# curioloop/rafting

Measured on AMD Instinct MI355X. Metric: raft-group decisions/sec (AppendEntries+vote), higher is better.
Workload: dtype int64

## Files before the change

### rafting_amd/csrc/rg_step.hpp

```cpp
#pragma once
#include "rg_device.hpp"
#include "rg_tier1n.hpp"

namespace rg {

typedef uint32_t u32x2 __attribute__((vector_size(8)));
typedef uint32_t u32x4 __attribute__((vector_size(16)));

template <class T> __device__ __forceinline__ T nt_load16(const T *p)
{
    static_assert(sizeof(T) == 16, "16-byte row");
    const u32x4 v = __builtin_nontemporal_load(reinterpret_cast<const u32x4 *>(p));
    T r; __builtin_memcpy(&r, &v, 16); return r;
}
template <class T> __device__ __forceinline__ T nt_load8(const T *p)
{
    static_assert(sizeof(T) == 8, "8-byte row");
    const u32x2 v = __builtin_nontemporal_load(reinterpret_cast<const u32x2 *>(p));
    T r; __builtin_memcpy(&r, &v, 8); return r;
}
template <class T> __device__ __forceinline__ void nt_store16(T *p, const T &x)
{
    static_assert(sizeof(T) == 16, "16-byte row");
    u32x4 v; __builtin_memcpy(&v, &x, 16);
// ... 535 lines not shown
                      c = (int64_t)sh_ev[slot][EV_C][lane], d = (int64_t)sh_ev[slot][EV_D][lane];
        int64_t e0 = (int64_t)(int32_t)aux;
        if constexpr (!EV32) e0 = (int64_t)sh_ev[slot][EV_E0][lane];
        const uint32_t kind = RG_HDR_KIND(hdr);
        { const int64_t top = *sh_flush; *sh_flush = ((kind == RG_EV_LOG_FLUSH) & (a > top)) ? a : top; }
        const bool skip = blocked & (kind != RG_EV_NONE);
        const bool done = tier1<F, int64_t, PeersWide<F>>(p, g, pe, st.fx, FAST & !skip, hdr, aux, a, b, c, d, e0);
        bool slow = !done & !skip;
        if (skip) st.fx = Fx{0u, RG_SKIPPED_AFTER_NEED_HOST, 0, 0};
        if (__builtin_amdgcn_ballot_w64(slow) != 0) {
            if (slow) slow = !tier15w<F, int64_t, PeersWide<F>>(p, g, pe, st.fx, FAST, hdr, aux, EV32 ? false : ((RG_HDR_HINT(hdr) != 0) & (p.hint != nullptr)), a, b, c, d, e0);
            if (slow) {
                int64_t hx = 0, hy = 0, e1 = e0, e2 = e0, e3 = e0;
                if constexpr (!EV32) {
                    hx = (int64_t)sh_ev[slot][EV_HX][lane]; hy = (int64_t)sh_ev[slot][EV_HY][lane];
                    e1 = (int64_t)sh_ev[slot][EV_E1][lane]; e2 = (int64_t)sh_ev[slot][EV_E2][lane]; e3 = (int64_t)sh_ev[slot][EV_E3][lane];
                }
                const Entries en = entries_of<EV32>(p, hdr, aux, e0, e1, e2, e3);
                const bool hinted = EV32 ? false : ((RG_HDR_HINT(hdr) != 0) & (p.hint != nullptr));
                st.run(hdr, aux, a, b, c, d, hinted, hx, hy, en, entries_readable(p, en, aux, RG_HDR_N(hdr)));
            }
        }
        const uint32_t status = st.fx.status, flags = st.fx.flags;
        if (status == RG_NEED_HOST) blocked = true;
        const uint32_t flags_all = flags | ((uint32_t)g.role << RG_F_ROLE_SHIFT) | (status << RG_F_STATUS_SHIFT);
        sh_out[slot][OUT_RESP][lane] = (flags & RG_F_REPLIED) ? (uint64_t)st.fx.resp_term : 0ull;
        sh_out[slot][OUT_FLAGS][lane] = (uint64_t)flags_all | ((uint64_t)g.role_epoch << 32);
        sh_out[slot][OUT_COMMIT][lane] = (uint64_t)g.commit;
        sh_out[slot][OUT_FROM][lane] = (uint64_t)st.fx.log_from;
        sh_out[slot][OUT_TERM][lane] = (uint64_t)g.term;
        sh_out[slot][OUT_VOTE][lane] = (uint64_t)(uint32_t)g.voted_for | ((uint64_t)(uint32_t)g.role << 32);
        lds_barrier();
    }
    uint32_t gi_out = gi;
    RG_FRESH_VGPR(gi_out);
    if (active) store_group(p.t, gi_out, g, pe, F);
    if (const int64_t at = sh_flush[1]; at != 0) {
        RG_GLOBAL_AS int64_t *slot = reinterpret_cast<RG_GLOBAL_AS int64_t *>((uint64_t)at);
        const int64_t top = sh_flush[0], window = sh_flush[2];
        if (top - window > *slot) *slot = top - window;
    }
}

template <int F, bool SPARSE>
__global__ __launch_bounds__(2 * BLOCK) void step_split_kernel(const StepParams p)
{
    __shared__ alignas(16) unsigned char smem[SplitLds<F, false>::BYTES];
    split_body<F, SPARSE, false>(p, smem);
}

struct Row32 { U32x2 h; I32x4 q; };

constexpr int CW_AUXC = 18;
template <int F = 0>
__device__ __forceinline__ uint32_t class_entry(const StepParams &p, uint32_t idx)
{
    const uint32_t kind = idx & 15u, slot = idx >> 4;
    const uint32_t P = (uint32_t)p.cluster, self = (uint32_t)p.self;
    const bool peer_ok = (slot < P) & (slot != self);
    const bool ack = (kind == RG_EV_AE_ACK) & peer_ok, vreq = (kind == RG_EV_RV_REQ) | (kind == RG_EV_PV_REQ),
               vrep = (kind == RG_EV_RV_REPLY) | (kind == RG_EV_PV_REPLY);
    const uint32_t j = ack ? (slot < self ? slot : slot - 1u) : 0u;
    const uint32_t cls = (ack ? 1u << CW_ACK : 0u) | (((kind == RG_EV_AE_REQ) & (slot < P)) ? 1u << CW_AE : 0u) | ((kind == RG_EV_CLIENT_APPEND) ? 1u << CW_CLIENT : 0u) |
                         (((ack | (kind == RG_EV_IS_ACK)) & peer_ok) ? 1u << CW_ACKANY : 0u) |
                         ((kind - (uint32_t)RG_EV_RV_REQ <= (uint32_t)(RG_EV_TIMEOUT - RG_EV_RV_REQ)) ? 1u << CW_ELK : 0u) |
                         ((vrep & peer_ok) ? 1u << CW_VR : 0u) | ((kind == RG_EV_PV_REPLY) ? 1u << CW_PV : 0u) | ((kind == RG_EV_TIMEOUT) ? 1u << CW_TO : 0u) |
                         ((vreq & (slot < P)) ? 1u << CW_VQ : 0u) | ((kind == RG_EV_PV_REQ) ? 1u << CW_PVQ : 0u) | ((kind == RG_EV_NONE) ? 1u << CW_NONE : 0u) |
                         ((((0x1CCu >> kind) & 1u) != 0) ? 1u << CW_AUXC : 0u);
    const uint32_t j4 = F > 6 ? (j & 15u) : j;
    return cls | (j4 << 10) | (slot << 5) | (31u - j);
}
__device__ __forceinline__ I32x4 class_word(const uint32_t *lutc, const Row32 &x)
{
    const uint32_t hdr = x.h.x, aux = x.h.y;
    const uint32_t e = lutc[hdr & 0xFFu];
    const int32_t n = (int32_t)(hdr >> 12);
    const sw same = (int32_t)(hdr << (31 - 10));
    const int32_t n_lim = (same >> 31) & (int32_t)RG_MAX_AE_ENTRIES;
    const sw ae_bad = ~s_pos(x.q.z) | s_lt(n_lim, n), cli_bad = s_lt(n, 1);
    const uint32_t auxm = (uint32_t)(((int32_t)(e << (31 - CW_AUXC)) | ((int32_t)(e << (31 - CW_AE)) & same)) >> 31);
    const uint32_t w = (uint32_t)x.q.x | (uint32_t)x.q.y | (uint32_t)x.q.z | (uint32_t)x.q.w | (aux & auxm);
    const uint32_t ood = (uint32_t)((int32_t)(w | (w << 1)) >> 31);
    const uint32_t off = (((uint32_t)ae_bad & 0x80000000u) >> (31 - CW_AE)) | (((uint32_t)cli_bad & 0x80000000u) >> (31 - CW_CLIENT)) | (1u << CW_AUXC) |
                         (ood & 0xFFF80000u);
    const uint32_t cw = (e & ~off) | ((hdr & 0x100u) << (CW_FLAG - 8));
    return I32x4{(int32_t)cw, (int32_t)aux, n, (int32_t)(hdr | (ood & KIND_OUT_OF_DOMAIN))};
}
__device__ __forceinline__ uint32_t expand_by_table(const uint32_t *lutm, const uint16_t *lute, uint32_t w)
{
    const uint32_t fast = lutm[w & 127u] | (uint32_t)lute[(w >> 7) & 127u];
    return ((int32_t)w < 0) ? (w & 0x00FFFFFFu) : fast;
}

template <int F, bool SPARSE, bool OUT32, int IOW = 1, int RPB = 1>
__device__ __forceinline__ bool narrow_body(const StepParams &p, unsigned char *smem)
{
    static_assert(RPB == 1 || (RPB == 2 && IOW == 1), "two rounds per hand-over: the two-wavefront workgroup only");
    constexpr int NO = 2 * RPB;
    typedef SplitLds<F, true, NO> L;
    I32x4 *sh_rec = reinterpret_cast<I32x4 *>(smem + L::N_REC);
    int32_t *sh_mv = reinterpret_cast<int32_t *>(smem + L::N_MV);
    I32x4 (*sh_evh)[BLOCK] = reinterpret_cast<I32x4 (*)[BLOCK]>(smem + L::N_EVH);
    I32x4 (*sh_evq)[BLOCK] = reinterpret_cast<I32x4 (*)[BLOCK]>(smem + L::N_EVQ);
    I32x4 (*sh_o0)[BLOCK] = reinterpret_cast<I32x4 (*)[BLOCK]>(smem + L::N_O0);
    I32x4 (*sh_o1)[BLOCK] = reinterpret_cast<I32x4 (*)[BLOCK]>(smem + L::N_O1);
    uint32_t *sh_bail = reinterpret_cast<uint32_t *>(smem + L::N_BAIL);
    uint32_t *sh_lutc = reinterpret_cast<uint32_t *>(smem + L::N_LUTC), *sh_lutm = reinterpret_cast<uint32_t *>(smem + L::N_LUTM);
    uint16_t *sh_lute = reinterpret_cast<uint16_t *>(smem + L::N_LUTE);
    uint32_t *sh_luts = reinterpret_cast<uint32_t *>(smem + L::N_LUTS);

    const uint32_t lane = threadIdx.x & (BLOCK - 1);
    const bool io_wave = __builtin_amdgcn_readfirstlane(threadIdx.x) >= (uint32_t)BLOCK;
    const uint32_t i = blockIdx.x * BLOCK + lane;
    const bool active = i < p.count;
    const uint32_t ir = active ? i : p.count - 1u;
    const uint32_t last_round = p.rounds - 1u;

    if (io_wave) {
        RG_HWID_BEGIN(1);
        const bool do_pub = IOW == 1 || __builtin_amdgcn_readfirstlane(threadIdx.x) < 2u * BLOCK;
        const bool do_ret = IOW == 1 || !do_pub;
        uint64_t b_head = reinterpret_cast<uint64_t>(p.head), b_q = reinterpret_cast<uint64_t>(p.abcd32),
                 b_reply = OUT32 ? reinterpret_cast<uint64_t>(p.out32) : reinterpret_cast<uint64_t>(p.reply),
                 b_logfx = reinterpret_cast<uint64_t>(p.logfx),
                 b_persist = OUT32 ? reinterpret_cast<uint64_t>(p.persist32) : reinterpret_cast<uint64_t>(p.persist);
        RG_OWN_SGPRS(b_head); RG_OWN_SGPRS(b_q); RG_OWN_SGPRS(b_reply); RG_OWN_SGPRS(b_logfx); RG_OWN_SGPRS(b_persist);
        const uint64_t round_rows = SPARSE ? p.stride : p.count;
        const uint32_t irm = ir & 0x0FFFFFFFu;
        int64_t io_base = 0;
        if constexpr (!OUT32) io_base = (p.has_bases != 0) ? p.t.ibase[SPARSE ? p.gid[ir] : ir] : 0;
        auto fetch = [&](uint32_t r, Row32 &x) {
            const uint64_t rb = (uint64_t)(r < p.rounds ? r : last_round) * round_rows;
            x.h = nt_load_at<U32x2>(b_head + rb * 8u, irm);
            x.q = nt_load_at<I32x4>(b_q + rb * 16u, irm);
        };
#pragma unroll
        for (int k = 0; k < 4; k++) sh_lutc[lane + 64u * k] = class_entry<F>(p, lane + 64u * k);
#pragma unroll
        for (int k = 0; k < 2; k++) {
            const uint32_t i7 = lane + 64u * k;
            sh_lutm[i7] = expand_predicates(i7);
            sh_lute[i7] = (uint16_t)(expand_predicates((i7 << 7) | 0x42u) & 0xFFFFu);
        }
        sh_luts[lane] = Tally::status_entry(lane);
        __builtin_amdgcn_wave_barrier();
        auto publish = [&](uint32_t slot, const Row32 &x) {
            sh_evh[slot][lane] = class_word(sh_lutc, x);
            sh_evq[slot][lane] = x.q;
        };
        Tally tally;
        auto retire = [&](uint32_t r, uint32_t hdr) {
            const uint32_t slot = r & (uint32_t)(NO - 1);
            const uint64_t rb16 = (uint64_t)r * round_rows * 16u;
            const I32x4 o0 = sh_o0[slot][lane], o1 = sh_o1[slot][lane];
            const uint32_t flags_all = expand_by_table(sh_lutm, sh_lute, (uint32_t)o0.y) | ((uint32_t)o1.w << RG_F_ROLE_SHIFT), flags = flags_all & 0xFFFFu, status = RG_F_STATUS(flags_all);
            if constexpr (OUT32) {
                nt_store_at(b_reply + rb16, irm, I32x4{(flags & RG_F_REPLIED) ? o0.x : 0, (int32_t)flags_all, o0.w, o1.x});
                if ((flags & RG_F_PERSIST) != 0) nt_store_at(b_persist + rb16, irm, I32x4{o1.y, o1.z, o0.z, o1.w});
            } else {
                rg_reply_t rep;
                rep.resp_term = (flags & RG_F_REPLIED) ? (int64_t)(uint32_t)o0.x : 0; rep.flags = flags_all; rep.role_epoch = (uint32_t)o0.z;
                nt_store_at(b_reply + rb16, irm, rep);
                const bool w_lfx = ((flags & (RG_F_COMMIT | RG_F_LOG_APPEND | RG_F_LOG_TRUNC)) != 0) | (status == RG_NEED_HOST);
                if (w_lfx) nt_store_at(b_logfx + rb16, irm, I64x2{to_abs((int64_t)(uint32_t)o0.w, io_base), to_abs((int64_t)(uint32_t)o1.x, io_base)});
                if ((flags & RG_F_PERSIST) != 0) {
                    rg_persist_t per;
                    per.term = (int64_t)(uint32_t)o1.y; per.voted_for = o1.z; per.role = o1.w;
                    nt_store_at(b_persist + rb16, irm, per);
                }
            }
            tally.add_packed_lut(RG_HDR_KIND(hdr), flags, status, sh_luts);
        };
        Row32 buf[4];
        uint32_t hdr_m1 = 0u, hdr_0, hdr_1;
        if (do_pub) {
            Row32 e0, e1;
            fetch(0, e0); fetch(1, e1); fetch(2, buf[2]); fetch(3, buf[3]); fetch(4, buf[0]); fetch(5, buf[1]);
            publish(0u, e0); publish(1u, e1);
            hdr_0 = e0.h.x; hdr_1 = e1.h.x;
        } else {
            hdr_0 = hdr_1 = 0u;
            for (int k = 0; k < 4; k++) { buf[k].h = U32x2{0u, 0u}; buf[k].q = I32x4{0, 0, 0, 0}; }
        }
        lds_barrier();
        { const uint32_t seen0 = *sh_bail; if (__builtin_amdgcn_readfirstlane(seen0) == 1u) return false; }
        bool bailed = false;
        uint32_t seen = 0u;
        RG_PROBE_BEGIN();
        if constexpr (RPB == 2) {
            uint32_t hk[4] = {hdr_0, hdr_1, 0u, 0u};
            for (uint32_t r0 = 0; r0 < p.rounds && !bailed; r0 += 4u) {
                if ((r0 & 127u) == 124u) tally.spill();
#pragma unroll
                for (int k = 0; k < 4; k++) {
                    const uint32_t r = r0 + (uint32_t)k;
                    if (r >= p.rounds) break;
                    Row32 &x = buf[(k + 2) & 3];
                    publish((r + 2u) & 3u, x);
                    RG_PROBE_MARK(0);
                    if (r >= 2u) retire(r - 2u, hk[(k + 2) & 3]);
                    hk[(k + 2) & 3] = x.h.x;
                    fetch(r + 6u, x);
                    RG_PROBE_MARK(1);
                    if ((k & 1) != 0 || r == last_round) {
                        const uint32_t mark = __builtin_amdgcn_readfirstlane(seen), pair = r >> 1;
                        if ((mark != 0u) & (mark <= pair + 1u)) { bailed = true; break; }
                        lds_barrier();
                        RG_PROBE_MARK(2);
                        seen = *sh_bail;
                    }
                }
            }
            if (bailed) return false;
            { const uint32_t mark = __builtin_amdgcn_readfirstlane(seen); if (mark != 0u) return false; }
            for (uint32_t q = p.rounds >= 2u ? p.rounds - 2u : 0u; q < p.rounds; q++) {
                const uint32_t i = q & 3u;
                retire(q, i == 0u ? hk[0] : (i == 1u ? hk[1] : (i == 2u ? hk[2] : hk[3])));
            }
            tally.spill();
#if defined(RG_PROBE)
            RG_PROBE_FLUSH(0);
#elif defined(RG_PROBE_HWID)
            RG_HWID_END(1);
#else
            tally.flush(p, lane, active);
#endif
            return true;
        }
        for (uint32_t r0 = 0; r0 < p.rounds && !bailed; r0 += 4u) {
            if ((r0 & 127u) == 124u) tally.spill();
#pragma unroll
            for (int k = 0; k < 4; k++) {
                const uint32_t r = r0 + (uint32_t)k;
                if (r >= p.rounds) break;
                Row32 &x = buf[(k + 2) & 3];
                if (do_pub) publish((r + 2u) & 3u, x);
                RG_PROBE_MARK(0);
                if constexpr (IOW == 1) {
                    if (r > 0) retire(r - 1u, hdr_m1);
                    hdr_m1 = hdr_0; hdr_0 = hdr_1; hdr_1 = x.h.x;
                } else {
                    if (do_ret && r > 0) retire(r - 1u, (uint32_t)sh_evh[(r - 1u) & 3u][lane].w);
                }
                if (do_pub) fetch(r + 6u, x);
                RG_PROBE_MARK(1);
                const uint32_t mark = __builtin_amdgcn_readfirstlane(seen);
                if ((mark != 0u) & (mark <= r + 1u)) { bailed = true; break; }
                lds_barrier();
                RG_PROBE_MARK(2);
                seen = *sh_bail;
            }
        }
        if (bailed) return false;
        { const uint32_t mark = __builtin_amdgcn_readfirstlane(seen); if (mark != 0u) return false; }
        if constexpr (IOW == 1) retire(last_round, hdr_m1);
        else if (do_ret) retire(last_round, (uint32_t)sh_evh[last_round & 3u][lane].w);
        tally.spill();
#if defined(RG_PROBE)
        if (do_pub) RG_PROBE_FLUSH(0);
#elif defined(RG_PROBE_HWID)
        if (do_pub) RG_HWID_END(1);
#else
        if (do_ret) tally.flush(p, lane, active);
#endif
        return true;
    }

    __builtin_amdgcn_s_setprio(3);
    RG_HWID_BEGIN(0);
    const uint32_t gi = SPARSE ? p.gid[ir] : ir;
    GroupN g;
    PeersNarrow<F> pe;
    int64_t *sh_base = reinterpret_cast<int64_t *>(smem + L::N_BASE) + lane;
    pe.rec = sh_rec + lane; pe.mv = sh_mv + lane * 4; pe.overflow = false; pe.base = 0;
    const bool FAST = p.fast_paths != 0;
    bool in_domain, any_base;
    {
        const int64_t base = (p.has_bases != 0) ? p.t.ibase[gi] : 0;
        any_base = __builtin_amdgcn_ballot_w64(base != 0) != 0;
        *sh_base = base;
        pe.base = base;
        Group g64;
        load_group(p.t, gi, g64);
        g64.s1 = g64.rc > 1 ? g64.s1 : 0; g64.s2 = g64.rc > 2 ? g64.s2 : 0; g64.s3 = g64.rc > 3 ? g64.s3 : 0;
        if (any_base) g64 = group_to_rel(g64, base);
        in_domain = fits32(g64, EV_LIMIT) & small_fields_fit(g64) & (p.force_wide == 0) & (p.rounds < (1u << 24)) & ((base == 0) | (g64.epoch_index > 0)) & (base >= 0);
        narrow_into(g, g64);
        g.nallow = FAST ? 0 : -1;
        g.recache();
        in_domain = in_domain & stage_peers<F>(p.t, gi, g64.prepared, pe);
    }
    bool bailed = __builtin_amdgcn_ballot_w64(!in_domain) != 0;
    if (lane == 0) *sh_bail = bailed ? 1u : 0u;
    bool blocked = false;
    int32_t flush_max = 0;
    lds_barrier();
    if (bailed) return false;
    RG_PROBE_BEGIN();
#ifdef RG_EVENT_PREFETCH
    I32x4 h_next = sh_evh[0][lane], q_next = sh_evq[0][lane];
#endif
    auto round = [&](const uint32_t r) {
#ifdef RG_EVENT_PREFETCH
        const I32x4 h = h_next, q = q_next;
#else
        const I32x4 h = sh_evh[r & 3u][lane], q = sh_evq[r & 3u][lane];
#endif
        RG_PROBE_MARK(0);
        OutN out;
        const sw done = tier1n<F>(p, g, pe, out, h.x, (uint32_t)h.y, h.z, q.x, q.y, q.z, q.w);
        const bool open = done >= 0;
        RG_PROBE_MARK(1);
        const uint64_t b_open = __builtin_amdgcn_ballot_w64(open);
        const uint32_t slot = r & (uint32_t)(NO - 1);
        sh_o0[slot][lane] = I32x4{out.resp, (int32_t)out.pw, (int32_t)g.role_epoch, g.commit};
        sh_o1[slot][lane] = I32x4{out.log_from, g.term, g.voted_for, g.role};
        if (b_open != 0) {
            const uint32_t hdr = ((uint32_t)h.w & ~(7u << 9)) | ((((uint32_t)h.w & RG_HDR_SAME_TERM) != 0) ? HDR_SAME_IN : 0u), aux = (uint32_t)h.y, kind = RG_HDR_KIND(hdr);
            const bool skip = open & blocked & (kind != RG_EV_NONE);
            flush_max = (open & (kind == RG_EV_LOG_FLUSH) & (q.x > flush_max)) ? q.x : flush_max;
            bool park;
            const bool slow = open & !skip & !tier15<F>(p, g, pe, out, park, open & !skip, h.x, h.y, h.z, q.x, q.y, q.z, q.w);
            if (park) { blocked = true; g.nallow = -1; g.recache(); }
            RG_NOTE_SLOW(slow, lane == 0);
            bool bail = (slow | (skip & (p.auto_window != 0))) & (kind == KIND_OUT_OF_DOMAIN);
            if (slow & !bail) {
                const int64_t base = any_base ? *sh_base : 0;
                pe.base = base;
                Group g64 = group_to_abs(widen(g), base);
                Stepper<F, PeersNarrow<F>> st(p, g64, pe);
                const Entries en = entries_of<true>(p, hdr, aux, 0, 0, 0, 0);
                const uint32_t ix = index_fields(kind);
                st.run(hdr, aux, (ix & 1u) ? to_abs(q.x, base) : (int64_t)q.x, (ix & 2u) ? to_abs(q.y, base) : (int64_t)q.y,
                       (ix & 4u) ? to_abs(q.z, base) : (int64_t)q.z, (ix & 8u) ? to_abs(q.w, base) : (int64_t)q.w, false, 0, 0, en, entries_readable(p, en, aux, RG_HDR_N(hdr)));
                g64 = group_to_rel(g64, base);
                st.fx.log_from = to_rel(st.fx.log_from, base);
                bail = !fits32(g64, STATE_LIMIT) | !small_fields_fit(g64) | pe.overflow | ((base != 0) & (g64.epoch_index <= 0)) |
                       (((uint64_t)st.fx.resp_term | (uint64_t)st.fx.log_from) >= (uint64_t)STATE_LIMIT);
                narrow_into(g, g64);
                if (st.fx.status == RG_NEED_HOST) blocked = true;
                g.nallow = (FAST & !blocked) ? 0 : -1;
                g.recache();
                out.pw = PW_SLOW | st.fx.flags | (st.fx.status << RG_F_STATUS_SHIFT);
                out.resp = (int32_t)st.fx.resp_term; out.log_from = (int32_t)st.fx.log_from;
            }
            if (skip) { out.pw = PW_SLOW | ((uint32_t)RG_SKIPPED_AFTER_NEED_HOST << RG_F_STATUS_SHIFT); out.resp = 0; out.log_from = 0; }
            if (__builtin_amdgcn_ballot_w64(bail) != 0) {
                if (lane == 0) *sh_bail = r / (uint32_t)RPB + 2u;
                bailed = true;
            }
            sh_o0[slot][lane] = I32x4{out.resp, (int32_t)out.pw, (int32_t)g.role_epoch, g.commit};
            sh_o1[slot][lane] = I32x4{out.log_from, g.term, g.voted_for, g.role};
        } else {
            RG_NOTE_SLOW(false, lane == 0);
        }
        RG_PROBE_MARK(2);
#ifdef RG_EVENT_PREFETCH
        h_next = sh_evh[(r + 1u) & 3u][lane]; q_next = sh_evq[(r + 1u) & 3u][lane];
#endif
        if constexpr (RPB == 1) {
            lds_barrier();
            RG_PROBE_MARK(3);
        }
    };
    if constexpr (RPB == 2) {
        for (uint32_t r = 0; r < p.rounds; r++) {
            round(r);
            if (bailed) break;
            if ((r & 1u) != 0u || r == last_round) {
                lds_barrier();
                RG_PROBE_MARK(3);
            }
        }
        if (bailed) lds_barrier();
    } else {
#ifdef RG_EVENT_PREFETCH
    { uint32_t r = 0; do { round(r); r++; } while (!bailed & (r < p.rounds)); }
#else
    for (uint32_t r = 0; r < p.rounds; r++) {
        round(r);
        if (bailed) break;
    }
#endif
    }
    if (bailed) return false;
    RG_PROBE_FLUSH(4);
    RG_HWID_END(0);
    if (active) {
        Group g64 = widen(g);
        pe.base = 0;
        if (any_base) {
            const int64_t base = *sh_base;
            pe.base = base;
            g64 = group_to_abs(g64, base);
        }
        uint32_t gi_out = gi;
        RG_FRESH_VGPR(gi_out);
        store_group(p.t, gi_out, g64, pe, F);
        if (p.auto_window != 0) {
            const int64_t base = *sh_base;
            advance_base(p, gi_out, base, to_abs(flush_max, base));
        }
    }
    return true;
}

#ifndef RG_NOTE_FALLBACK
#define RG_NOTE_FALLBACK() ((void)0)
#endif

#ifndef RG_ROUNDS_PER_HANDOVER
#define RG_ROUNDS_PER_HANDOVER 1
#endif
template <int F, bool SPARSE, int WAVES, bool OUT32, int IOW = 1>
__global__ __launch_bounds__((1 + IOW) * BLOCK) __attribute__((amdgpu_waves_per_eu(WAVES, 8))) void step32_kernel(const StepParams p)
{
    constexpr int RPB = (WAVES == 1 && IOW == 1) ? RG_ROUNDS_PER_HANDOVER : 1;
    __shared__ alignas(16) unsigned char smem[SplitLds<F, true, 2 * RPB>::BYTES];
    if (narrow_body<F, SPARSE, OUT32, IOW, RPB>(p, smem)) return;
    if (threadIdx.x == 0) { RG_NOTE_FALLBACK(); atomicAdd(p.wide_bodies, 1ull); }
    if constexpr (IOW == 2) {
        if (__builtin_amdgcn_readfirstlane(threadIdx.x) >= 2u * BLOCK) {
            for (uint32_t k = 0; k < p.rounds + 2u; k++) lds_barrier();
            return;
        }
    }
    lds_barrier();
    split_body<F, SPARSE, true, OUT32>(p, smem);
}

template <int F, bool SPARSE, int WAVES, bool OUT32>
__global__ __launch_bounds__(2 * BLOCK) __attribute__((amdgpu_waves_per_eu(WAVES, 8))) void step32_wide_kernel(const StepParams p)
{
    __shared__ alignas(16) unsigned char smem[SplitLds<F, true>::BYTES];
    if (threadIdx.x == 0) { RG_NOTE_FALLBACK(); atomicAdd(p.wide_bodies, 1ull); }
    split_body<F, SPARSE, true, OUT32>(p, smem);
}

#if !defined(RG_BUILD_ONLY_F4)
#define RG_F_MASK 0x7FFEu
#elif defined(RG_BUILD_ALSO_F)
#define RG_F_MASK ((1u << 4) | (RG_BUILD_ALSO_F))
#else
#define RG_F_MASK (1u << 4)
#endif

#if !defined(RG_TU) || RG_TU == 1
#define RG_TU_MAIN 1
#endif

template <class L, int F>
static hipError_t launch_one(const L &l)
{
    if constexpr (((RG_F_MASK) >> F) & 1u) return l.template run<F>();
    else return hipErrorInvalidValue;
}
template <class L, int LO>
hipError_t launch_range(const L &l, int followers)
{
    switch (followers - LO) {
    case 0: return launch_one<L, LO>(l);
    case 1: return launch_one<L, LO + 1>(l);
    case 2: return launch_one<L, LO + 2>(l);
    case 3: return launch_one<L, LO + 3>(l);
    default: return hipErrorInvalidValue;
    }
}
template <class L>
static hipError_t launch_followers(const L &l, int followers)
{
    switch (followers) {
    case 1: return launch_one<L, 1>(l);
    case 2: return launch_one<L, 2>(l);
    case 3: return launch_one<L, 3>(l);
    case 4: return launch_one<L, 4>(l);
    case 5: return launch_one<L, 5>(l);
    case 6: return launch_one<L, 6>(l);
    case 7: case 8: case 9: case 10: return launch_range<L, 7>(l, followers);
    case 11: case 12: case 13: case 14: return launch_range<L, 11>(l, followers);
    default: return hipErrorInvalidValue;
    }
}

template <class Fn>
static hipError_t lift(bool b, Fn fn) { return b ? fn(std::true_type{}) : fn(std::false_type{}); }

template <int F> constexpr int WAVES_MANY = F <= 6 ? 4 : 1;
constexpr uint32_t MANY_BLOCKS = 1024u;
#ifdef RG_IOW2
constexpr int SMALL_IOW = 2;
#else
constexpr int SMALL_IOW = 1;
#endif

template <int F, bool SPARSE, bool OUT32>
static hipError_t launch_compact(const StepParams &p, hipStream_t s)
{
    const uint32_t blocks = (p.count + BLOCK - 1) / BLOCK;
    if (p.count >= (1u << 28)) return hipErrorInvalidValue;
    constexpr int MANY = WAVES_MANY<F>, IOW = (F <= 6 && OUT32 && !SPARSE) ? SMALL_IOW : 1;
    const bool many = blocks > MANY_BLOCKS;
    const dim3 grid(blocks), wg(2 * BLOCK);
    if (p.force_wide != 0) {
        if (many) hipLaunchKernelGGL((step32_wide_kernel<F, SPARSE, MANY, OUT32>), grid, wg, 0, s, p);
        else      hipLaunchKernelGGL((step32_wide_kernel<F, SPARSE, 1, OUT32>), grid, wg, 0, s, p);
// ... 31 lines not shown
```

### rafting_amd/csrc/rg_tier1n.hpp

```cpp
#pragma once
#include "rg_device.hpp"

namespace rg {

typedef int32_t sw;

__device__ __forceinline__ sw s_lt(int32_t x, int32_t y) { return (int32_t)((uint32_t)x - (uint32_t)y); }
__device__ __forceinline__ sw s_ne(int32_t x, int32_t y) { return (int32_t)(((uint32_t)x ^ (uint32_t)y) + 0x7FFFFFFFu); }
__device__ __forceinline__ sw s_pos(int32_t x) { return (int32_t)(0u - (uint32_t)x); }
__device__ __forceinline__ sw s_nz(int32_t x) { return (int32_t)((uint32_t)x | (0u - (uint32_t)x)); }
__device__ __forceinline__ uint32_t push_bit(uint32_t acc, sw w) { return (acc << 1) | ((uint32_t)w >> 31); }

constexpr int CW_ACK = 31;
constexpr int CW_AE = 30;
constexpr int CW_CLIENT = 29;
constexpr int CW_ACKANY = 28;
constexpr int CW_FLAG = 27;
constexpr int CW_ELK = 26;
constexpr int CW_VR = 25;
constexpr int CW_PV = 24;
constexpr int CW_TO = 23;
constexpr int CW_VQ = 22;
constexpr int CW_PVQ = 21;
constexpr int CW_NONE = 19;
__device__ __forceinline__ sw cw_bit(int32_t cw, int bit) { return (int32_t)((uint32_t)cw << (31 - bit)); }
template <int F> __device__ __forceinline__ uint32_t cw_follower(int32_t cw) { return ((uint32_t)cw >> 10) & (F <= 6 ? 7u : 15u); }

constexpr uint32_t PW_SLOW = 1u << 31;
__device__ __forceinline__ uint32_t expand_predicates(uint32_t w)
{
    auto m = [&](int bit) { return (uint32_t)((int32_t)(w << (31 - bit)) >> 31); };
    const uint32_t fa = ~m(6), contains = ~m(5), conv = m(4) | m(10), app = m(3), commit = m(2), hb = ~m(1) | m(9), drop = m(0);
    const uint32_t vq = m(13), succ = (fa & contains) | m(12), reset = fa | m(11) | conv, to_pre = m(8), cand = m(7);
    const uint32_t fast = (succ & RG_F_SUCCESS) | ((fa | vq) & RG_F_REPLIED) | (conv & (RG_F_PERSIST | RG_F_ROLE_CHANGED)) | (reset & RG_F_RESET_TIMER) |
                          (commit & RG_F_COMMIT) | (app & RG_F_LOG_APPEND) | (hb & (RG_EMIT_HEARTBEAT << RG_F_EMIT_SHIFT)) |
                          (to_pre & (RG_EMIT_PREVOTE << RG_F_EMIT_SHIFT)) | (cand & (RG_EMIT_REQVOTE << RG_F_EMIT_SHIFT)) |
                          (drop & ((uint32_t)RG_DROPPED_STALE_ROLE << RG_F_STATUS_SHIFT));
    return (w & PW_SLOW) ? (w & 0x00FFFFFFu) : fast;
}

struct GroupN {
    int32_t term, commit, epoch_index, epoch_term, first, last, elected_term;
    int32_t s0, s1, s2, s3, t0, t1, t2, t3, lt, top;
    int32_t voted_for, leader, votes, role, rc;
    uint32_t role_epoch, elected_epoch, pending;
    sw td, prepared, log_dirty, peers_dirty;
    sw nallow;
    sw stf_n, stl_n, stc_n;

    __device__ __forceinline__ void recache()
    {
        const int32_t r = role, n = rc, l = last, e = epoch_index;
        const sw na = nallow, pr = prepared;
        const sw not_l = s_ne(r, RG_LEADER), no_log = s_lt(n, 1);
        stf_n = na | s_pos(r) | pr | no_log | ~s_lt(e, l);
        stl_n = na | not_l | ~pr;
        stc_n = na | not_l | no_log;
    }
    __device__ __forceinline__ void push_run(int32_t index, int32_t t)
    {
        int n = rc;
        int32_t x0 = s0, x1 = s1, x2 = s2, x3 = s3, y0 = t0, y1 = t1, y2 = t2, y3 = t3;
        const int32_t f = first, cur_lt = lt, cur_top = top;
        const bool empty = n == 0;
        const bool newrun = empty | (cur_lt != t);
        const bool shift = newrun & (n == K);
        x0 = shift ? x1 : x0; y0 = shift ? y1 : y0;
        x1 = shift ? x2 : x1; y1 = shift ? y2 : y1;
        x2 = shift ? x3 : x2; y2 = shift ? y3 : y2;
        n = shift ? K - 1 : n;
        const bool w0 = newrun & (n == 0), w1 = newrun & (n == 1), w2 = newrun & (n == 2), w3 = newrun & (n == 3);
        x0 = w0 ? index : x0; y0 = w0 ? t : y0;
        x1 = w1 ? index : x1; y1 = w1 ? t : y1;
        x2 = w2 ? index : x2; y2 = w2 ? t : y2;
        x3 = w3 ? index : x3; y3 = w3 ? t : y3;
        n += newrun ? 1 : 0;
        s0 = x0; s1 = x1; s2 = x2; s3 = x3; t0 = y0; t1 = y1; t2 = y2; t3 = y3;
        lt = t; top = newrun ? index : cur_top;
        rc = n;
        first = empty ? index : f;
        log_dirty = -1;
    }
};

__device__ __forceinline__ Group widen(const GroupN &n)
{
    Group g;
    g.term = n.term; g.commit = n.commit; g.epoch_index = n.epoch_index; g.epoch_term = n.epoch_term; g.first = n.first; g.last = n.last;
    g.elected_term = n.elected_term;
    g.s0 = n.s0; g.s1 = n.s1; g.s2 = n.s2; g.s3 = n.s3; g.t0 = n.t0; g.t1 = n.t1; g.t2 = n.t2; g.t3 = n.t3; g.lt = n.lt; g.top = n.top;
    g.voted_for = n.voted_for; g.leader = n.leader; g.votes = n.votes; g.role = n.role; g.rc = n.rc;
    g.role_epoch = n.role_epoch; g.elected_epoch = n.elected_epoch; g.pending = n.pending;
    g.td = n.td < 0; g.prepared = n.prepared < 0; g.log_dirty = n.log_dirty < 0; g.peers_dirty = n.peers_dirty < 0;
    return g;
}
__device__ __forceinline__ void narrow_into(GroupN &n, const Group &g)
{
    n.term = (int32_t)g.term; n.commit = (int32_t)g.commit; n.epoch_index = (int32_t)g.epoch_index; n.epoch_term = (int32_t)g.epoch_term;
    n.first = (int32_t)g.first; n.last = (int32_t)g.last; n.elected_term = (int32_t)g.elected_term;
    n.s0 = (int32_t)g.s0; n.s1 = (int32_t)g.s1; n.s2 = (int32_t)g.s2; n.s3 = (int32_t)g.s3;
    n.t0 = (int32_t)g.t0; n.t1 = (int32_t)g.t1; n.t2 = (int32_t)g.t2; n.t3 = (int32_t)g.t3; n.lt = (int32_t)g.lt; n.top = (int32_t)g.top;
    n.voted_for = g.voted_for; n.leader = g.leader; n.votes = g.votes; n.role = g.role; n.rc = g.rc;
    n.role_epoch = g.role_epoch; n.elected_epoch = g.elected_epoch; n.pending = g.pending;
    n.td = g.td ? -1 : 0; n.prepared = g.prepared ? -1 : 0; n.log_dirty = g.log_dirty ? -1 : 0; n.peers_dirty = g.peers_dirty ? -1 : 0;
}
__device__ __forceinline__ bool small_fields_fit(const Group &g)
{
    const uint32_t w = g.role_epoch | g.elected_epoch | (uint32_t)g.votes | (uint32_t)(g.leader + 1) | (uint32_t)(g.voted_for + 1);
    return (w < EV_LIMIT) & ((uint32_t)g.role <= (uint32_t)RG_LEADER);
}

struct OutN {
    uint32_t pw;
    int32_t resp;
    int32_t log_from;
};

template <int F>
__device__ __forceinline__ sw tier1n(const StepParams &p, GroupN &g, PeersNarrow<F> &pe, OutN &out, int32_t cw, uint32_t aux_u, int32_t n,
                                     int32_t a, int32_t b, int32_t c, int32_t d)
{
    const int32_t aux = (int32_t)aux_u;
    const int32_t term = g.term, last = g.last, commit = g.commit, epoch = g.epoch_index, lt = g.lt, top = g.top;
    const int32_t role = g.role, rc = g.rc, leader = g.leader, votes = g.votes, voted = g.voted_for;
    const int32_t repoch = (int32_t)g.role_epoch;
    const sw td = g.td, prep = g.prepared, nallow = g.nallow, stl_n = g.stl_n;
    const int32_t slot = (int32_t)(((uint32_t)cw >> 5) & 15u);
    const sw flg = cw_bit(cw, CW_FLAG);
    const sw x_ta = s_lt(term, a);
    const sw x_aux = s_ne(aux, repoch);
    const sw x_tl = s_ne(lt, term);
    const uint32_t j = cw_follower<F>(cw);
    const I32x4 st = pe.rec[j * BLOCK];
    int32_t m[F];
    pe.load_matches(m);
    __builtin_amdgcn_sched_barrier(0);

    const sw x_ct = s_ne(c, lt);
    const sw rf = x_ta | td;
    const bool contains = x_ct >= 0;
    const int32_t n_eff = contains ? n : 0;
    const int32_t ae_last = last + n_eff;
    const int32_t ae_x = vmin<int32_t>(d, ae_last);
    const sw x_de = s_lt(epoch, d);
    const sw fa_n = (~cw_bit(cw, CW_AE) | g.stf_n | s_lt(a, term)) | ((s_ne(leader, slot) & ~rf) | s_ne(b, last)) |
                    (~x_ct & x_de & s_lt(ae_x, commit));
    const bool m_fa = fa_n >= 0;
    const sw ae_ref = ~fa_n & rf;
    const bool m_ref = ae_ref < 0;
    const sw ae_wc = ~fa_n & ~x_ct & x_de;
    const sw app_ae = ~fa_n & s_pos(n_eff);

    __builtin_amdgcn_sched_barrier(0);
    const int32_t s_epoch = st.x, s_next = st.y, s_match = st.z, s_rej = st.w;
    const sw pend = (int32_t)(g.pending << ((uint32_t)cw & 31u));
    const sw adv = flg & s_lt(s_match, c);
    const bool m_adv = adv < 0;
    const int32_t n_match = m_adv ? c : s_match;
    const int32_t n_next = m_adv ? (int32_t)((uint32_t)c + 1u) : s_next;
#pragma unroll
    for (int i = 0; i < F; i++) m[i] = (j == (uint32_t)i) ? n_match : m[i];
    int32_t full, major;
    major_indices<F, int32_t>(m, full, major);
    const sw lookup = flg & s_pos(major);
    const sw bad_major = lookup & (s_lt(rc, 1) | s_lt(major, top) | s_lt(last, major));
    const int32_t ct0 = (lt == term) ? major : full;
    const sw rollback = lookup & s_pos(ct0) & s_lt(ct0, commit);
    const sw fk_n = (~cw | stl_n | x_aux) | (x_ta | s_ne(b, s_epoch) | pend) | (s_lt(c, s_match) | (~flg & ~s_pos(s_match))) |
                    (~s_lt(b, n_next) | bad_major | rollback);
    const bool m_fk = fk_n >= 0;
    const bool m_ct = (~fk_n & lookup) < 0;
    const int32_t ack_ct = m_ct ? ct0 : 0;
    const sw ackany = cw_bit(cw, CW_ACKANY) & ~nallow;
    const sw drop = ackany & x_aux;

    const int32_t last_n = last + n;
    const sw fc_n = ~cw_bit(cw, CW_CLIENT) | g.stc_n | ~s_lt(last_n, (int32_t)STATE_LIMIT);
    const bool m_fc = fc_n >= 0;

    pe.store_ack(j, s_epoch, m_fk ? n_next : s_next, m_fk ? n_match : s_match, m_fk ? ((flg < 0) ? 0 : (int32_t)((uint32_t)s_rej + 1u)) : s_rej);
    g.term = m_fa ? a : term;
    g.role_epoch = (uint32_t)repoch + (m_ref ? 1u : 0u);
    g.td = td & ~ae_ref;
    g.votes = m_ref ? 1 : votes;
    g.leader = m_fa ? slot : leader;
    g.last = m_fa ? ae_last : (m_fc ? last_n : last);
    const sw app = app_ae | ~fc_n;
    g.log_dirty = g.log_dirty | app;
    g.peers_dirty = g.peers_dirty | ~fk_n;
    const int32_t cand = (ae_wc < 0) ? ae_x : ack_ct;
    const int32_t new_commit = vmax<int32_t>(commit, cand);
    g.commit = new_commit;
    uint32_t pw = push_bit(0u, fa_n);
    pw = push_bit(pw, x_ct);
    pw = push_bit(pw, ae_ref);
    pw = push_bit(pw, app);
    pw = push_bit(pw, s_lt(commit, new_commit));
    pw = push_bit(pw, fc_n);
    out.resp = a;
    out.log_from = last + 1;
    sw done = ~fa_n | ~fk_n | ~fc_n | drop | cw_bit(cw, CW_NONE);
    sw any_drop = drop;
    uint32_t pw_el = 0u;

    const sw x_pl = s_ne(aux, lt);
    const sw rare = (app_ae & x_pl) | (~fc_n & (x_tl | ~prep));
    const sw ack_down = ackany & ~x_aux & ~stl_n & x_ta;
    const sw election = (cw_bit(cw, CW_ELK) & ~nallow) | ack_down;
    const uint64_t b_rare = __builtin_amdgcn_ballot_w64(rare < 0), b_el = __builtin_amdgcn_ballot_w64(election < 0);
    if ((b_rare | b_el) != 0) {
        if (b_rare != 0) {
            const bool ae_newrun = (app_ae & x_pl) < 0, fc_newrun = (~fc_n & x_tl) < 0, fc_prepare = (~fc_n & ~prep) < 0;
            if (ae_newrun | fc_newrun) g.push_run(last + 1, ae_newrun ? aux : term);
            if (fc_prepare) {
                pe.store_prepare(epoch, last + 2);
                g.pending = 0;
                g.prepared = -1; g.peers_dirty = -1;
            }
        }
        if (b_el != 0) {
            const int32_t term1 = term + 1;
            const sw is_pv = cw_bit(cw, CW_PV);
            const sw not_f = s_pos(role), not_c = s_ne(role, RG_CANDIDATE), not_l = s_ne(role, RG_LEADER);
            sw conv = ack_down, conv_self = 0, to_c = 0, win_rv = 0, late_higher = 0, count = 0, el_fast = ack_down;
            sw to_pre = 0, to_lead = 0, resp_own = 0, no_vote = 0;
            const sw vr_shape = cw_bit(cw, CW_VR) & ~nallow;
            const sw to_kind = cw_bit(cw, CW_TO) & ~nallow & (s_pos(aux) | ~s_nz(p.require_fence));
            const sw vq_shape = cw_bit(cw, CW_VQ) & ~nallow;
            const uint64_t b_vr = __builtin_amdgcn_ballot_w64(vr_shape < 0), b_to = __builtin_amdgcn_ballot_w64(to_kind < 0), b_vq = __builtin_amdgcn_ballot_w64(vq_shape < 0);
            if (b_vr != 0) {
                const int32_t el_term = g.elected_term, el_epoch = (int32_t)g.elected_epoch;
                const sw sender_bad = (is_pv & (not_f | ~td)) | (~is_pv & not_c);
                const int32_t T = (is_pv < 0) ? term1 : term;
                const sw vr_cur = vr_shape & ~x_aux & ~sender_bad;
                const sw x_Ta = s_lt(T, a);
                const sw vr_grant = vr_cur & ~x_Ta & flg;
                const sw vr_win = vr_grant & ~s_lt(votes + 1, p.majority);
                const sw x_lt = s_lt(el_term, a);
                const sw late = vr_shape & ~is_pv & x_aux & (s_pos(el_epoch) & ~s_ne(aux, el_epoch));
                const sw late_noop = late & ~x_lt & (~flg | s_lt(el_term, term) | (~s_ne(el_term, term) & ~not_l));
                const sw vote_drop = vr_shape & x_aux & ~late;
                late_higher = late & x_lt;
                win_rv = vr_win & ~is_pv;
                conv_self = vr_win;
                to_c = vr_win & is_pv;
                count = vr_grant & ~vr_win;
                conv = conv | (vr_cur & x_Ta) | vr_win | (late_higher & ~s_lt(a, term));
                el_fast = el_fast | vr_cur | late_higher | late_noop | vote_drop;
                any_drop = any_drop | vote_drop;
                pw_el = (uint32_t)to_c >> 31;
            }
            if (b_to != 0) {
                const sw to_stale = to_kind & s_pos(aux) & x_aux;
                const sw to_live = to_kind & ~to_stale;
                const sw pre = s_nz(p.pre_vote);
                const sw to_cand = to_live & ((~not_f & ~pre) | ~not_c);
                to_pre = to_live & ~not_f & pre;
                to_lead = to_live & ~not_l;
                conv_self = conv_self | to_cand;
                to_c = to_c | to_cand;
                conv = conv | to_cand | to_pre;
                el_fast = el_fast | to_kind;
                any_drop = any_drop | to_stale;
                const uint32_t lead_bit = (uint32_t)to_lead >> 31;
                pw_el = pw_el | (lead_bit << 4) | push_bit(push_bit(lead_bit, to_pre), to_cand);
            }
            if (b_vq != 0) {
                const sw is_pvq = cw_bit(cw, CW_PVQ);
                const sw vq = vq_shape & ~not_f & ~s_lt(g.rc, 1);
                const sw utd = s_lt(lt, c) | (~s_ne(c, lt) & ~s_lt(b, last));
                const sw pv_judge = vq & is_pvq & x_ta & td;
                const sw rv_same = vq & ~is_pvq & ~x_ta & ~s_lt(a, term);
                const sw voted_other = s_ne(voted, slot) | voted;
                const sw rv_new = vq & ~is_pvq & x_ta;
                const sw vq_success = ((pv_judge | rv_new) & utd) | (rv_same & ~voted_other);
                no_vote = rv_new & ~utd;
                resp_own = vq & ~rv_new;
                conv = conv | rv_new;
                el_fast = el_fast | vq;
                pw_el = pw_el | (push_bit(push_bit(push_bit(0u, vq), vq_success), pv_judge) << 4);
            }
            const sw lead_prepare = to_lead & ~g.prepared;
            const uint64_t b_conv = __builtin_amdgcn_ballot_w64((conv | lead_prepare | late_higher) < 0);
            const int32_t votes_counted = g.votes + (int32_t)((uint32_t)count >> 31);
            out.resp = (resp_own < 0) ? term : a;
            pw_el = pw_el | (((uint32_t)conv >> 28) & 8u);
            done = done | el_fast;
            g.votes = votes_counted;
            if (b_conv != 0) {
                const bool m_conv = conv < 0, m_winrv = win_rv < 0;
                const int32_t new_role = (win_rv < 0) ? RG_LEADER : ((to_c < 0) ? RG_CANDIDATE : RG_FOLLOWER);
                const int32_t new_term = (to_c < 0) ? term1 : (((win_rv | to_pre) < 0) ? term : a);
                const int32_t new_vote = (conv_self < 0) ? p.self : ((to_pre < 0) ? voted : ((no_vote < 0) ? RG_NO_NODE : slot));
                if (lead_prepare < 0) {
                    pe.store_prepare(epoch, ((g.rc > 0) ? last : epoch) + 1);
                    g.pending = 0;
                }
                g.elected_epoch = m_winrv ? (uint32_t)repoch : ((late_higher < 0) ? 0u : g.elected_epoch);
                g.elected_term = m_winrv ? term : g.elected_term;
                g.term = m_conv ? new_term : g.term;
                g.role = m_conv ? new_role : g.role;
                g.voted_for = m_conv ? new_vote : g.voted_for;
                g.role_epoch = g.role_epoch + (m_conv ? 1u : 0u);
                g.td = (g.td & ~conv) | to_pre;
                g.votes = m_conv ? 1 : votes_counted;
                g.leader = m_conv ? RG_NO_NODE : g.leader;
                g.prepared = (g.prepared & ~conv) | lead_prepare;
                g.peers_dirty = g.peers_dirty | lead_prepare;
            }
        }
        g.recache();
    }
    pw = push_bit(pw, any_drop);
    out.pw = pw | (pw_el << 7);
    return done;
}

template <int F>
__device__ __forceinline__ bool tier15(const StepParams &p, GroupN &g, PeersNarrow<F> &pe, OutN &out, bool &park, const bool open, const int32_t cw,
                                       const int32_t aux, const int32_t n, const int32_t a, const int32_t b, const int32_t c, const int32_t d)
{
    bool fixed = false;
    {
        const int32_t slot = (int32_t)(((uint32_t)cw >> 5) & 15u);
        const uint32_t j = cw_follower<F>(cw);
        const bool nack_shape = open & (cw_bit(cw, CW_ACK) < 0) & (cw_bit(cw, CW_FLAG) >= 0) & (g.stl_n >= 0) & (aux == (int32_t)g.role_epoch) & (a <= g.term);
        if (nack_shape) {
            const I32x4 st = pe.rec[j * BLOCK];
            const bool pend = ((g.pending >> j) & 1u) != 0;
            if ((st.z == 0) & (b == st.x) & !pend) {
                const int32_t rej = (int32_t)((uint32_t)st.w + 1u);
                const int32_t next = vmax<int32_t>(st.y - (int32_t)rejection_step(rej), b + 1);
                const int32_t s_next = vmin<int32_t>(st.y - 1, next);
                pe.store_ack(j, st.x, s_next, 0, rej);
                g.pending = g.pending | ((s_next <= b) ? (1u << j) : 0u);
                g.peers_dirty = -1;
                out.pw = PW_SLOW;
                out.resp = 0; out.log_from = 0;
                fixed = true;
            }
        }
        const bool cand_vq = open & (cw_bit(cw, CW_VQ) < 0) & (g.nallow >= 0) & (g.role == RG_CANDIDATE) & (g.term < a) & (slot != p.self);
        if (cand_vq) {
            g.role = RG_FOLLOWER; g.term = a; g.voted_for = slot;
            g.role_epoch = g.role_epoch + 1u;
            g.td = 0; g.leader = RG_NO_NODE; g.votes = 1; g.prepared = 0;
            g.recache();
            out.pw = PW_SLOW | RG_F_PERSIST | RG_F_ROLE_CHANGED | RG_F_RESET_TIMER | RG_F_REPLIED | RG_F_SUCCESS;
            out.resp = a; out.log_from = 0;
            fixed = true;
        }
    }
    {
        const bool miss = open & (cw_bit(cw, CW_AE) < 0) & (g.stf_n >= 0) & (a >= g.term) & (g.epoch_index < b) & (b <= g.last) & (b < g.s0);
        if (miss) {
            out.pw = PW_SLOW | ((uint32_t)RG_NEED_HOST << RG_F_STATUS_SHIFT);
            out.resp = 0;
            out.log_from = b;
        }
        park = miss;
        fixed = fixed | miss;
        if (__builtin_amdgcn_ballot_w64(open & !fixed) == 0) return fixed;
    }
    const int32_t term = g.term, last = g.last, commit = g.commit, epoch = g.epoch_index, lt = g.lt, top = g.top;
    const int32_t slot = (int32_t)(((uint32_t)cw >> 5) & 15u);
    const bool refresh = (term < a) | (g.td < 0);
    const int32_t new_last = b + n;
    const int32_t commit_to = vmin<int32_t>(d, new_last);
    const bool with_commit = epoch < d;
    const bool ok = open & (cw_bit(cw, CW_AE) < 0) & (g.stf_n >= 0) & (a >= term) & ((g.leader == slot) | refresh) &
                    (b < last) & (b >= top) & (b > epoch) & (c == lt) & (n >= 1) & (aux != lt) & (b >= commit) & !(with_commit & (commit_to < commit));
    if (ok) {
        g.term = a;
        g.role_epoch = g.role_epoch + (refresh ? 1u : 0u);
        g.td = 0;
        g.votes = refresh ? 1 : g.votes;
        g.leader = slot;
        g.last = b;
        g.push_run(b + 1, aux);
        g.last = new_last;
        const int32_t new_commit = with_commit ? vmax<int32_t>(commit, commit_to) : commit;
        g.commit = new_commit;
        out.pw = PW_SLOW | RG_F_RESET_TIMER | RG_F_REPLIED | RG_F_SUCCESS | RG_F_LOG_TRUNC | RG_F_LOG_APPEND |
                 (refresh ? (RG_F_PERSIST | RG_F_ROLE_CHANGED) : 0u) | ((new_commit > commit) ? RG_F_COMMIT : 0u);
        out.resp = a;
        out.log_from = b + 1;
    }
    return ok | fixed;
}

}
```

Before: 64.07 billion.

## Repack staged output slots so retire stores rows directly and packs role into pw

Reorders the two per-round LDS staging vectors so the first is nearly the reply row and the second is exactly the persist row. On the 32-bit output path, retire can then store them with little reassembly, and the role now travels in high bits of the predicate word instead of a separate read. The header ring for the one-writer path becomes a 4-entry array shared with the two-round path, and the tier-1 predicate word is assembled with the election bits merged earlier. Some election-path values are now reread from the group state, and the run push uses the updated term. This could subtly change semantics if those values differed from the earlier locals.

```diff
diff --git a/rafting_amd/csrc/rg_step.hpp b/rafting_amd/csrc/rg_step.hpp
--- a/rafting_amd/csrc/rg_step.hpp
+++ b/rafting_amd/csrc/rg_step.hpp
@@ -711,34 +711,36 @@
         auto retire = [&](uint32_t r, uint32_t hdr) {
             const uint32_t slot = r & (uint32_t)(NO - 1);
             const uint64_t rb16 = (uint64_t)r * round_rows * 16u;
-            const I32x4 o0 = sh_o0[slot][lane], o1 = sh_o1[slot][lane];
-            const uint32_t flags_all = expand_by_table(sh_lutm, sh_lute, (uint32_t)o0.y) | ((uint32_t)o1.w << RG_F_ROLE_SHIFT), flags = flags_all & 0xFFFFu, status = RG_F_STATUS(flags_all);
+            I32x4 o0 = sh_o0[slot][lane];
+            const uint32_t flags_all = expand_by_table(sh_lutm, sh_lute, (uint32_t)o0.y) | (((uint32_t)o0.y >> (PW_ROLE_SHIFT - RG_F_ROLE_SHIFT)) & RG_F_ROLE_MASK),
+                           flags = flags_all & 0xFFFFu, status = RG_F_STATUS(flags_all);
             if constexpr (OUT32) {
-                nt_store_at(b_reply + rb16, irm, I32x4{(flags & RG_F_REPLIED) ? o0.x : 0, (int32_t)flags_all, o0.w, o1.x});
-                if ((flags & RG_F_PERSIST) != 0) nt_store_at(b_persist + rb16, irm, I32x4{o1.y, o1.z, o0.z, o1.w});
+                o0.x = (flags & RG_F_REPLIED) ? o0.x : 0; o0.y = (int32_t)flags_all;
+                nt_store_at(b_reply + rb16, irm, o0);
+                if ((flags & RG_F_PERSIST) != 0) nt_store_at(b_persist + rb16, irm, sh_o1[slot][lane]);
             } else {
+                const I32x4 o1 = sh_o1[slot][lane];
                 rg_reply_t rep;
-                rep.resp_term = (flags & RG_F_REPLIED) ? (int64_t)(uint32_t)o0.x : 0; rep.flags = flags_all; rep.role_epoch = (uint32_t)o0.z;
+                rep.resp_term = (flags & RG_F_REPLIED) ? (int64_t)(uint32_t)o0.x : 0; rep.flags = flags_all; rep.role_epoch = (uint32_t)o1.z;
                 nt_store_at(b_reply + rb16, irm, rep);
                 const bool w_lfx = ((flags & (RG_F_COMMIT | RG_F_LOG_APPEND | RG_F_LOG_TRUNC)) != 0) | (status == RG_NEED_HOST);
-                if (w_lfx) nt_store_at(b_logfx + rb16, irm, I64x2{to_abs((int64_t)(uint32_t)o0.w, io_base), to_abs((int64_t)(uint32_t)o1.x, io_base)});
+                if (w_lfx) nt_store_at(b_logfx + rb16, irm, I64x2{to_abs((int64_t)(uint32_t)o0.z, io_base), to_abs((int64_t)(uint32_t)o0.w, io_base)});
                 if ((flags & RG_F_PERSIST) != 0) {
                     rg_persist_t per;
-                    per.term = (int64_t)(uint32_t)o1.y; per.voted_for = o1.z; per.role = o1.w;
+                    per.term = (int64_t)(uint32_t)o1.x; per.voted_for = o1.y; per.role = o1.w;
                     nt_store_at(b_persist + rb16, irm, per);
                 }
             }
             tally.add_packed_lut(RG_HDR_KIND(hdr), flags, status, sh_luts);
         };
         Row32 buf[4];
-        uint32_t hdr_m1 = 0u, hdr_0, hdr_1;
+        uint32_t hk[4] = {0u, 0u, 0u, 0u};
         if (do_pub) {
             Row32 e0, e1;
             fetch(0, e0); fetch(1, e1); fetch(2, buf[2]); fetch(3, buf[3]); fetch(4, buf[0]); fetch(5, buf[1]);
             publish(0u, e0); publish(1u, e1);
-            hdr_0 = e0.h.x; hdr_1 = e1.h.x;
+            hk[0] = e0.h.x; hk[1] = e1.h.x;
         } else {
-            hdr_0 = hdr_1 = 0u;
             for (int k = 0; k < 4; k++) { buf[k].h = U32x2{0u, 0u}; buf[k].q = I32x4{0, 0, 0, 0}; }
         }
         lds_barrier();
@@ -747,7 +749,6 @@
         uint32_t seen = 0u;
         RG_PROBE_BEGIN();
         if constexpr (RPB == 2) {
-            uint32_t hk[4] = {hdr_0, hdr_1, 0u, 0u};
             for (uint32_t r0 = 0; r0 < p.rounds && !bailed; r0 += 4u) {
                 if ((r0 & 127u) == 124u) tally.spill();
 #pragma unroll
@@ -796,8 +797,8 @@
                 if (do_pub) publish((r + 2u) & 3u, x);
                 RG_PROBE_MARK(0);
                 if constexpr (IOW == 1) {
-                    if (r > 0) retire(r - 1u, hdr_m1);
-                    hdr_m1 = hdr_0; hdr_0 = hdr_1; hdr_1 = x.h.x;
+                    if (r > 0) retire(r - 1u, hk[(k + 3) & 3]);
+                    hk[(k + 2) & 3] = x.h.x;
                 } else {
                     if (do_ret && r > 0) retire(r - 1u, (uint32_t)sh_evh[(r - 1u) & 3u][lane].w);
                 }
@@ -812,7 +813,7 @@
         }
         if (bailed) return false;
         { const uint32_t mark = __builtin_amdgcn_readfirstlane(seen); if (mark != 0u) return false; }
-        if constexpr (IOW == 1) retire(last_round, hdr_m1);
+        if constexpr (IOW == 1) { const uint32_t i = last_round & 3u; retire(last_round, i == 0u ? hk[0] : (i == 1u ? hk[1] : (i == 2u ? hk[2] : hk[3]))); }
         else if (do_ret) retire(last_round, (uint32_t)sh_evh[last_round & 3u][lane].w);
         tally.spill();
 #if defined(RG_PROBE)
@@ -872,8 +873,8 @@
         RG_PROBE_MARK(1);
         const uint64_t b_open = __builtin_amdgcn_ballot_w64(open);
         const uint32_t slot = r & (uint32_t)(NO - 1);
-        sh_o0[slot][lane] = I32x4{out.resp, (int32_t)out.pw, (int32_t)g.role_epoch, g.commit};
-        sh_o1[slot][lane] = I32x4{out.log_from, g.term, g.voted_for, g.role};
+        sh_o0[slot][lane] = I32x4{out.resp, (int32_t)(out.pw | ((uint32_t)g.role << PW_ROLE_SHIFT)), g.commit, out.log_from};
+        sh_o1[slot][lane] = I32x4{g.term, g.voted_for, (int32_t)g.role_epoch, g.role};
         if (b_open != 0) {
             const uint32_t hdr = ((uint32_t)h.w & ~(7u << 9)) | ((((uint32_t)h.w & RG_HDR_SAME_TERM) != 0) ? HDR_SAME_IN : 0u), aux = (uint32_t)h.y, kind = RG_HDR_KIND(hdr);
             const bool skip = open & blocked & (kind != RG_EV_NONE);
@@ -908,8 +909,10 @@
                 if (lane == 0) *sh_bail = r / (uint32_t)RPB + 2u;
                 bailed = true;
             }
-            sh_o0[slot][lane] = I32x4{out.resp, (int32_t)out.pw, (int32_t)g.role_epoch, g.commit};
-            sh_o1[slot][lane] = I32x4{out.log_from, g.term, g.voted_for, g.role};
+            int32_t w_commit = g.commit, w_term = g.term, w_vote = g.voted_for, w_epoch = (int32_t)g.role_epoch, w_role = g.role;
+            RG_FRESH_VGPR(w_commit); RG_FRESH_VGPR(w_term); RG_FRESH_VGPR(w_vote); RG_FRESH_VGPR(w_epoch); RG_FRESH_VGPR(w_role);
+            sh_o0[slot][lane] = I32x4{out.resp, (int32_t)(out.pw | ((uint32_t)w_role << PW_ROLE_SHIFT)), w_commit, out.log_from};
+            sh_o1[slot][lane] = I32x4{w_term, w_vote, w_epoch, w_role};
         } else {
             RG_NOTE_SLOW(false, lane == 0);
         }
diff --git a/rafting_amd/csrc/rg_tier1n.hpp b/rafting_amd/csrc/rg_tier1n.hpp
--- a/rafting_amd/csrc/rg_tier1n.hpp
+++ b/rafting_amd/csrc/rg_tier1n.hpp
@@ -27,6 +27,7 @@
 template <int F> __device__ __forceinline__ uint32_t cw_follower(int32_t cw) { return ((uint32_t)cw >> 10) & (F <= 6 ? 7u : 15u); }
 
 constexpr uint32_t PW_SLOW = 1u << 31;
+constexpr int PW_ROLE_SHIFT = 24;
 __device__ __forceinline__ uint32_t expand_predicates(uint32_t w)
 {
     auto m = [&](int bit) { return (uint32_t)((int32_t)(w << (31 - bit)) >> 31); };
@@ -178,6 +179,8 @@
     const sw fc_n = ~cw_bit(cw, CW_CLIENT) | g.stc_n | ~s_lt(last_n, (int32_t)STATE_LIMIT);
     const bool m_fc = fc_n >= 0;
 
+    out.resp = a;
+    out.log_from = last + 1;
     pe.store_ack(j, s_epoch, m_fk ? n_next : s_next, m_fk ? n_match : s_match, m_fk ? ((flg < 0) ? 0 : (int32_t)((uint32_t)s_rej + 1u)) : s_rej);
     g.term = m_fa ? a : term;
     g.role_epoch = (uint32_t)repoch + (m_ref ? 1u : 0u);
@@ -189,19 +192,16 @@
     g.log_dirty = g.log_dirty | app;
     g.peers_dirty = g.peers_dirty | ~fk_n;
     const int32_t cand = (ae_wc < 0) ? ae_x : ack_ct;
-    const int32_t new_commit = vmax<int32_t>(commit, cand);
-    g.commit = new_commit;
+    const sw adv_commit = s_lt(commit, cand);
+    g.commit = vmax<int32_t>(commit, cand);
     uint32_t pw = push_bit(0u, fa_n);
     pw = push_bit(pw, x_ct);
     pw = push_bit(pw, ae_ref);
     pw = push_bit(pw, app);
-    pw = push_bit(pw, s_lt(commit, new_commit));
+    pw = push_bit(pw, adv_commit);
     pw = push_bit(pw, fc_n);
-    out.resp = a;
-    out.log_from = last + 1;
     sw done = ~fa_n | ~fk_n | ~fc_n | drop | cw_bit(cw, CW_NONE);
     sw any_drop = drop;
-    uint32_t pw_el = 0u;
 
     const sw x_pl = s_ne(aux, lt);
     const sw rare = (app_ae & x_pl) | (~fc_n & (x_tl | ~prep));
@@ -211,19 +211,22 @@
     if ((b_rare | b_el) != 0) {
         if (b_rare != 0) {
             const bool ae_newrun = (app_ae & x_pl) < 0, fc_newrun = (~fc_n & x_tl) < 0, fc_prepare = (~fc_n & ~prep) < 0;
-            if (ae_newrun | fc_newrun) g.push_run(last + 1, ae_newrun ? aux : term);
+            if (ae_newrun | fc_newrun) g.push_run(out.log_from, ae_newrun ? aux : g.term);
             if (fc_prepare) {
-                pe.store_prepare(epoch, last + 2);
+                pe.store_prepare(epoch, out.log_from + 1);
                 g.pending = 0;
                 g.prepared = -1; g.peers_dirty = -1;
             }
         }
         if (b_el != 0) {
+            const int32_t term = g.term, votes = g.votes, last = g.last, lt = g.lt, repoch = (int32_t)g.role_epoch;
+            const sw td = g.td;
             const int32_t term1 = term + 1;
             const sw is_pv = cw_bit(cw, CW_PV);
             const sw not_f = s_pos(role), not_c = s_ne(role, RG_CANDIDATE), not_l = s_ne(role, RG_LEADER);
             sw conv = ack_down, conv_self = 0, to_c = 0, win_rv = 0, late_higher = 0, count = 0, el_fast = ack_down;
             sw to_pre = 0, to_lead = 0, resp_own = 0, no_vote = 0;
+            uint32_t pw_el = 0u;
             const sw vr_shape = cw_bit(cw, CW_VR) & ~nallow;
             const sw to_kind = cw_bit(cw, CW_TO) & ~nallow & (s_pos(aux) | ~s_nz(p.require_fence));
             const sw vq_shape = cw_bit(cw, CW_VQ) & ~nallow;
@@ -285,6 +288,7 @@
             const int32_t votes_counted = g.votes + (int32_t)((uint32_t)count >> 31);
             out.resp = (resp_own < 0) ? term : a;
             pw_el = pw_el | (((uint32_t)conv >> 28) & 8u);
+            pw = pw | (pw_el << 6);
             done = done | el_fast;
             g.votes = votes_counted;
             if (b_conv != 0) {
@@ -311,8 +315,7 @@
         }
         g.recache();
     }
-    pw = push_bit(pw, any_drop);
-    out.pw = pw | (pw_el << 7);
+    out.pw = push_bit(pw, any_drop);
     return done;
 }
 
```

Result: no change. 64.52 billion, median of 6 (+0.7%).
